# iaomw/Tracer

Hardware: AMD Instinct MI355X
Metric: Mrays/s at 1920x1080x64spp (higher is better)
Workload: dtype f32

## Files before the change

### include/tracer_test_hooks.h

```cpp
#ifndef TRACER_TEST_HOOKS_H
#define TRACER_TEST_HOOKS_H

#include "tracer_abi.h"

#ifdef __cplusplus
extern "C" {
#endif

trc_status trc_debug_profile(trc_ctx* ctx, uint64_t* out, uint32_t n_sites);
trc_status trc_sppm_hash_cells(trc_ctx* ctx, const float* cells , size_t n, float hash_scale, float* out );

trc_status trc_div_by_test(trc_ctx* ctx, const float* a, const float* b, size_t n, float* fast , float* plain );
trc_status trc_unary_test(trc_ctx* ctx, uint32_t op, uint32_t first_bits, uint64_t count, uint64_t* n_mismatch, uint32_t* first_mismatch);

trc_status trc_debug_denoise_state(trc_ctx* ctx, float* integrated, float* history, float* moments);

trc_status trc_texture_sample_test(trc_ctx* ctx, uint32_t index, const float* uv , size_t n, float* rgb );

trc_status trc_debug_env_tables(trc_ctx* ctx, float* weight, uint32_t* rows, uint32_t* marg, double* total, float* build_ms);
trc_status trc_env_light_test(trc_ctx* ctx, const uint32_t* draws , size_t n, float* dir_pdf ,
                              const float* dirs , size_t m, float* pdf );

trc_status trc_debug_mesh_light_tables(trc_ctx* ctx, uint32_t* alias , uint32_t* tri , float* pdfA ,
                                       double* total, uint32_t* n_lights);
trc_status trc_mesh_light_test(trc_ctx* ctx, const uint32_t* draws , const float* pos , size_t n, uint32_t* tri ,
                               float* out );

typedef struct trc_kernel_choice {
    uint32_t shape, variant, lds_resident, triangle_materials, strip, launches;
} trc_kernel_choice;
trc_status trc_debug_last_kernel(trc_ctx* ctx, trc_kernel_choice* out);


typedef struct trc_residency {
    uint32_t cu_count, block, waves, planned_per_cu, planned_with, per_cu;
    uint64_t lds_bytes;
    uint32_t lds_static_bytes, per_cu_block1280, dense_memo_rows, reserved;
} trc_residency;
trc_status trc_debug_last_residency(trc_ctx* ctx, trc_residency* out);

#ifdef __cplusplus
}
#endif
#endif
```

### tracer_amd/abi.py

```python
import ctypes as C

TRC_ABI_VERSION = 13
TRC_TILE = 16
TRC_MAX_BVH_DEPTH = 64
TREE_SAH, TREE_TRIANGLE_LEAVES = 1, 2
TRC_UNIQUE_ID_BYTES = 128
DT_U8, DT_U32, DT_F32 = 1, 3, 7
OP_SUM, OP_MAX, OP_MIN = 0, 2, 3

PRIM_SPHERE, PRIM_SQUARE, PRIM_CUBE, PRIM_TRIANGLE, PRIM_BVH, PRIM_UNKNOW = range(6)
(MAT_DIFFUSE, MAT_LAMBERT, MAT_ORENNAYAR, MAT_PLASTIC, MAT_METAL, MAT_GLASS,
 MAT_ISOTROPIC, MAT_DIELECTRIC, MAT_DEMOFOX, MAT_PBR, MAT_NIL) = range(11)
TEX_CONSTANT, TEX_CHECKER, TEX_NOISE, TEX_IMAGE = range(4)
INTEGRATOR_PATH, INTEGRATOR_MIS, INTEGRATOR_VOLUME = 0, 1, 2
MEDIUM_NIL, MEDIUM_HOMOGENEOUS, MEDIUM_GRIDDENSITY = 0, 1, 2
SCENE_CORNELL, SCENE_CORNELL_SPHERES, SCENE_CORNELL_MESH, SCENE_CORNELL_VOLUME = 0, 1, 2, 3
FLAG_COLLECT_STATS = 1
FLAG_FIXED_ORDER = 2
FLAG_SOBOL = 4
FLAG_SMALL_BLOCKS, FLAG_LARGE_BLOCKS = 8, 16
FLAG_ENV_LIGHT = 32
FLAG_MESH_LIGHTS = 64
TRACE_ANY_HIT, TRACE_PRODUCTION = 1, 2
SOBOL_DIMS, SOBOL_MATRIX_SIZE = 40, 52
# ... 174 lines not shown


class Hit(C.Structure):
    _fields_ = [("hit", C.c_int32), ("pType", C.c_int32), ("pIndex", C.c_uint32), ("t", C.c_float),
                ("p", C.c_float * 3), ("gn", C.c_float * 3), ("sn", C.c_float * 3), ("uv", C.c_float * 2),
                ("material", C.c_uint32), ("PDF", C.c_float),
                ("n_descend", C.c_uint32), ("n_return", C.c_uint32), ("n_leaf", C.c_uint32)]


class GBufferTexel(C.Structure):
    _fields_ = [("depth", C.c_float), ("normal", C.c_float * 3), ("albedo", C.c_float * 3), ("id", C.c_uint32)]


class DenoiseParams(C.Structure):
    _fields_ = [("flags", C.c_uint32), ("iterations", C.c_uint32), ("alpha_color", C.c_float), ("alpha_moments", C.c_float),
                ("sigma_z", C.c_float), ("normal_exponent", C.c_uint32), ("sigma_l", C.c_float), ("min_history", C.c_uint32)]


GBUFFER_MISS = 0xFFFFFFFF
DENOISE_DEMODULATE = 1
DENOISE_ALBEDO_EPS = 0.001
DENOISE_MAX_ITERATIONS = 5


class TreeCost(C.Structure):
    _fields_ = [("root_half_area", C.c_double), ("interior_half_area", C.c_double), ("leaf_half_area", C.c_double),
                ("n_interior", C.c_uint32), ("n_leaves", C.c_uint32)]


class KernelChoice(C.Structure):
    _fields_ = [("shape", C.c_uint32), ("variant", C.c_uint32), ("lds_resident", C.c_uint32), ("triangle_materials", C.c_uint32),
                ("strip", C.c_uint32), ("launches", C.c_uint32)]


class Residency(C.Structure):
    _fields_ = [("cu_count", C.c_uint32), ("block", C.c_uint32), ("waves", C.c_uint32), ("planned_per_cu", C.c_uint32),
                ("planned_with", C.c_uint32), ("per_cu", C.c_uint32), ("lds_bytes", C.c_uint64),
                ("lds_static_bytes", C.c_uint32), ("per_cu_block1280", C.c_uint32), ("dense_memo_rows", C.c_uint32), ("reserved", C.c_uint32)]


KERNEL_SHAPES = ("one", "strip", "pwg", "dense")
KERNEL_VARIANTS = ("plain", "stats", "sobol", "tex", "env", "env_tex", "mesh", "mesh_tex")


class LaunchShape(C.Structure):
    _fields_ = [("entries", C.c_uint32), ("wave_slots", C.c_uint32), ("longest_entry_ms", C.c_double),
                ("sum_entries_ms", C.c_double), ("work_over_slots_ms", C.c_double), ("clock_mhz", C.c_double)]


class Stats(C.Structure):
    _fields_ = [("paths", C.c_uint64), ("rays", C.c_uint64), ("shaded", C.c_uint64),
                ("n_descend", C.c_uint64), ("n_return", C.c_uint64),
                ("n_leaf_sphere", C.c_uint64), ("n_leaf_square", C.c_uint64),
                ("n_leaf_cube", C.c_uint64), ("n_leaf_triangle", C.c_uint64),
                ("n_hit_triangle", C.c_uint64), ("n_hit_cube", C.c_uint64),
                ("launches", C.c_uint64), ("kernel_ms", C.c_double), ("schedule_ms", C.c_double)]

    def as_dict(self):
        return {n: getattr(self, n) for n, _ in self._fields_}


_EXPECTED_SIZES = {float2: 8, float3: 16, float4x4: 64, AABB: 32, BVH: 64, Sphere: 272, Square: 272, Cube: 240,
                   TriangleVertex: 32, Pose: 144, SkinInfluence: 32, SkinBone: 128, MorphDelta: 24, TextureInfo: 32, Material: 64, Camera: 176, Ray: 32, Params: 32, GBufferTexel: 32, DenoiseParams: 32, TreeCost: 32,
                   PhotonRecord: 80, CameraRecord: 112, Complex: 96}
for _t, _n in _EXPECTED_SIZES.items():
    assert C.sizeof(_t) == _n, f"{_t.__name__}: ctypes size {C.sizeof(_t)} != ABI size {_n}"

DEVICE_SYMBOLS = [
    "trc_abi_version", "trc_build_flavor", "trc_has_test_hooks", "trc_status_string", "trc_last_error", "trc_create", "trc_destroy",
    "trc_upload_scene", "trc_upload_density", "trc_upload_scene_lbvh", "trc_upload_scene_sah", "trc_upload_scene_device", "trc_download_bvh", "trc_lbvh_info", "trc_set_camera", "trc_set_environment", "trc_set_environment_map", "trc_resize", "trc_seed",
    "trc_upload_rng", "trc_download_rng", "trc_upload_accum", "trc_download_accum", "trc_clear_accum", "trc_tonemap",
    "trc_render", "trc_synchronize", "trc_trace_rays", "trc_get_stats", "trc_reset_stats",
    "trc_sppm_init", "trc_sppm_frames", "trc_sppm_download",
    "trc_device_info", "trc_device_pci_bus_id", "trc_shard_seed", "trc_group_compose_samples", "trc_group_compose_samples_async", "trc_group_unique_id", "trc_group_init", "trc_group_reduce_accum", "trc_group_reduce_accum_async", "trc_group_allreduce_mean_accum", "trc_download_composed", "trc_group_finalize",
    "trc_group_set_collectives", "trc_debug_set", "trc_debug_block_costs", "trc_debug_launch_shape", "trc_debug_primary_replays",
    "trc_denoise_default_params", "trc_denoise", "trc_download_denoised", "trc_tonemap_denoised", "trc_download_gbuffer", "trc_denoise_reset",
    "trc_upload_textures", "trc_upload_triangle_materials", "trc_update_vertices", "trc_debug_refit_ms",
    "trc_pose_vertices", "trc_download_vertices", "trc_debug_pose_overflows", "trc_skin_bind", "trc_skin_vertices",
    "trc_morph_bind", "trc_morph_vertices", "trc_recompute_normals",
    "trc_rebuild_tree", "trc_tree_cost",
]
HOOK_SYMBOLS = ["trc_debug_profile", "trc_sppm_hash_cells", "trc_div_by_test", "trc_unary_test", "trc_debug_denoise_state", "trc_texture_sample_test",
                "trc_debug_env_tables", "trc_env_light_test", "trc_debug_mesh_light_tables", "trc_mesh_light_test", "trc_debug_last_kernel",
                "trc_debug_last_residency"]
HOST_SYMBOLS = [
    "trc_host_build_node", "trc_host_build_tree", "trc_host_tree_depth", "trc_host_make_camera",
    "trc_host_prepare_camera", "trc_host_fill_rng", "trc_host_scene_create", "trc_host_scene_create_leaves", "trc_host_scene_destroy",
    "trc_host_scene_view", "trc_host_scene_load_pbrt", "trc_host_mesh_load_obj", "trc_host_mesh_load_pbrt", "trc_host_mesh_load_ply", "trc_host_load_hdr", "trc_host_mesh_make_ball", "trc_host_mesh_replicate", "trc_host_mesh_from_arrays",
    "trc_host_mesh_view", "trc_host_mesh_destroy", "trc_host_make_density_info", "trc_host_make_cloud",
    "trc_host_load_density_pbrt", "trc_host_free", "trc_host_write_png", "trc_host_sobol_matrices32",
    "trc_host_sobol_interval_tables", "trc_host_load_png", "trc_host_scene_load_pbrt_flags", "trc_host_scene_triangle_materials",
]
```

### tracer_amd/csrc/dev_bsdf.hpp

```cpp
#pragma once

#include "dev_prof.hpp"
#include "dev_vec.hpp"

namespace trcdev {

TRC_DEV void coordinate_system(const F3 a, F3& b, F3& c) {
    if (fabsf(a.x) > fabsf(a.y)) b = f3(-a.z, 0, a.x);
    else b = f3(0, a.z, -a.y);
    b = normalize(b);
    c = cross(a, b);
}
TRC_DEV F2 concentric_sample_disk(const F2 u) {
    F2 uo; uo.x = 2.f * u.x - 1; uo.y = 2.f * u.y - 1;
    F2 r0; r0.x = 0; r0.y = 0;
    if (uo.x == 0 && uo.y == 0) return r0;
    const float PiOver2 = kPi / 2.0f, PiOver4 = kPi / 4.0f;
    const bool wide = fabsf(uo.x) > fabsf(uo.y);
    const float r = wide ? uo.x : uo.y;
    const float q = (wide ? uo.y : uo.x) / r;
    const float theta = wide ? PiOver4 * q : PiOver2 - PiOver4 * q;
    float s, c;
    dm_sincosf(theta, &s, &c);
    F2 out; out.x = r * c; out.y = r * s;
// ... 424 lines not shown
    const float etaA = 1.0f, etaB = 1.5f;
    bool live;
    bool pdf_live = false;
    bool f_live = false;
    F3 wi = wi_out, whA = wh, whB = wh;
    float eta = 0, fres_cos = 0, fres_eta = 1.5f;
    if (refl) {
        live = !(dot(wo, wh) <= 0);
        if (live) { wi = reflect(wo, wh); live = !(wo.z * wi.z <= 0); }
        if (live) {
            pdf_live = true;
            const float cosThetaO = abs_cos_theta(wo), cosThetaI = abs_cos_theta(wi);
            F3 sum = wi + wo;
            f_live = !(cosThetaI == 0 || cosThetaO == 0) && !(sum.x == 0 && sum.y == 0 && sum.z == 0);
            if (f_live) {
                whB = normalize(sum);
                const float d001 = whB.x * 0.0f + whB.y * 0.0f + whB.z * 1.0f;
                const F3 whf = (d001 < 0.f) ? -whB : whB;
                fres_cos = dot(wi, whf);
                fres_eta = 1.5f;
            }
        }
    } else {
        live = !(dot(wo, wh) < 0);
        if (live) live = refract(wo, wh, cos_theta(wo) > 0 ? (etaA / etaB) : (etaB / etaA), wi);
        if (live) {
            eta = cos_theta(wo) > 0 ? (etaB / etaA) : (etaA / etaB);
            const bool same_side = wo.z * wi.z > 0;
            whA = normalize(wo + wi * eta);
            const bool backfacing = dot(wo, whA) * dot(wi, whA) > 0;
            pdf_live = !same_side && !backfacing;
            whB = whA;
            if (whB.z < 0) whB = -whB;
            f_live = pdf_live && !(cos_theta(wi) == 0 || cos_theta(wo) == 0);
            fres_cos = dot(wo, whB);
            fres_eta = etaA;
        }
    }
    float D_A = 0, D_B = 0, lam_o = 0, lam_i = 0, fres = 0;
    if (pdf_live) {
        lam_o = d.lambda(wo);
        D_A = d.D(whA);
        D_B = D_A;
        if (refl && f_live) D_B = d.D(whB);
        if (f_live) {
            lam_i = d.lambda(wi);
            fres = fr_dielectric(fres_cos, fres_eta);
        }
    }
    F3 out = f3(0);
    if (live) {
        wi_out = wi;
        const float G1 = rcp1(1 + lam_o);
        const float G = rcp1(1 + lam_o + lam_i);
        if (refl) {
            const float dist_pdf = D_A * G1 * fabsf(dot(wo, wh)) / abs_cos_theta(wo);
            pdf_out = dist_pdf / (4 * dot(wo, wh));
            if (f_live) {
                const float cosThetaO = abs_cos_theta(wo), cosThetaI = abs_cos_theta(wi);
                out = f3(R) * D_B * G * f3(fres) / (4 * cosThetaI * cosThetaO);
            }
        } else {
            float p = 0;
            if (pdf_live) {
                const float sqrtDenom = dot(wo, whA) + eta * dot(wi, whA);
                const float dwh_dwi = fabsf((eta * eta * dot(wi, whA)) / (sqrtDenom * sqrtDenom));
                const float dist_pdf = D_A * G1 * fabsf(dot(wo, whA)) / abs_cos_theta(wo);
                p = dist_pdf * dwh_dwi;
            }
            pdf_out = p;
            if (f_live) {
                const float cosThetaO = cos_theta(wo), cosThetaI = cos_theta(wi);
                const float sqrtDenom = dot(wo, whB) + eta * dot(wi, whB);
                const float factor = 1;
                out = (f3(1.0f) - f3(fres)) * f3(0.98f) *
                      fabsf(D_B * G * eta * eta * fabsf(dot(wi, whB)) * fabsf(dot(wo, whB)) * factor * factor /
                            (cosThetaI * cosThetaO * sqrtDenom * sqrtDenom));
            }
        }
    }
    return out;
}

typedef MicroRefl<TrowbridgeReitzD<Alpha_01_02>, FrCond> MetalLobe;

constexpr int kMatDiffuse = 0, kMatLambert = 1, kMatPlastic = 3, kMatMetal = 4, kMatGlass = 5, kMatNil = 10;
constexpr int kTexConstant = 0, kTexChecker = 1, kTexImage = 3;

TRC_DEV F3 texture_value(int tex_type, F3 albedo, F2 uv) {
    if (tex_type == kTexChecker) {
        float s, c, s2, c2;
        dm_sincosf(8 * kPi * uv.x, &s, &c);
        dm_sincosf(kPi / 2 + 4 * kPi * uv.y, &s2, &c2);
        float sines = s * c2;
        return albedo * (0.5f * (sines < 0 ? 0.0f : 1.0f) + 0.5f);
    }
    return (tex_type >= 0 && tex_type <= 3) ? albedo : f3(1.0f);
}

template <bool STATS>
TRC_DEV F3 material_S_F(int type, F3 color, F3 wo, F3& wi, F2 uu, float& pdf, TravCounters& cnt) {
    const bool plastic = type == kMatPlastic, glass = type == kMatGlass;
    F3 out = f3(0);
    if (type == kMatMetal) {
        ProfScope<STATS> scope(cnt, kProfMetal);
        out = color * MetalLobe::S_F(1.0f, wo, wi, uu, pdf);
    } else if (type == kMatLambert || (plastic && uu.x < 0.5f)) {
        ProfScope<STATS> scope(cnt, kProfLambert);
        F2 u2 = uu;
        if (plastic) u2.x *= 2;
        const float v = Lambert::S_F(wo, wi, u2, pdf);
        out = plastic ? color * (f3(0.35f, 0.12f, 0.48f) * v) : color * f3(v);
    } else if (plastic || glass) {
        const float ratio = 0.25f;
        const bool refl = plastic || uu.x < ratio;
        F2 u2 = uu;
        if (plastic) { u2.x -= 0.5f; u2.x *= 2.0f; }
        else if (refl) u2.x = uu.x / ratio;
        else u2.x = (uu.x - ratio) / (1.0f - ratio);
        const Beckmann d = Beckmann::make_lobe(plastic);
        F3 lobe = f3(0);
        if (wo.z != 0) {
            F3 wh;
            { ProfScope<STATS> scope(cnt, kProfBeckSample); wh = d.sample_wh(wo, u2); }
            ProfScope<STATS> scope(cnt, kProfBeckEval);
            lobe = beckmann_finish(d, refl, plastic ? 1.0f : 0.98f, wo, wh, wi, pdf);
        }
        out = plastic ? color * (f3(0.2f) * lobe) : color * lobe;
    }
    return out;
}
TRC_DEV F3 material_S_F(int type, F3 color, F3 wo, F3& wi, F2 uu, float& pdf) {
    TravCounters none;
    return material_S_F<false>(type, color, wo, wi, uu, pdf, none);
}

TRC_DEV F3 material_F(int type, F3 color, F3 wo, F3 wi, F2 uu, float& pdf) {
    const bool plastic = type == kMatPlastic, glass = type == kMatGlass;
    if (type == kMatMetal) {
        pdf = MetalLobe::pdf(wo, wi);
        return color * MetalLobe::F(1.0f, wo, wi);
    }
    if (type == kMatLambert || (plastic && uu.x < 0.5f)) {
        pdf = Lambert::pdf(wo, wi);
        const float v = Lambert::F(wo, wi);
        return plastic ? color * (f3(0.35f, 0.12f, 0.48f) * v) : color * f3(v);
    }
    if (plastic || glass) {
        const float ratio = 0.25f;
        const Beckmann d = Beckmann::make_lobe(plastic);
        if (plastic || uu.x < ratio) {
            const float p = BeckRefl::pdf(d, wo, wi);
            pdf = plastic ? p : ratio * p;
            const F3 f = BeckRefl::F(d, plastic ? 1.0f : 0.98f, wo, wi);
            return plastic ? color * (f3(0.2f) * f) : color * f;
        }
        pdf = (1 - ratio) * BeckTransGlass::pdf(d, wo, wi);
        return color * BeckTransGlass::F(d, wo, wi);
    }
    pdf = 0;
    return f3(0);
}

}
```

### tracer_amd/csrc/trc_hooks.hip

```cpp
#include <hip/hip_runtime.h>

#include <string>

#include "trc_ctx.hpp"
#include "trc_render_config.hpp"

extern "C" int trc_has_test_hooks(void) {
#ifdef TRC_TEST_HOOKS
    return 1;
#else
    return 0;
#endif
}

#ifdef TRC_TEST_HOOKS
__global__ void __launch_bounds__(256) k_div_by_test(const float* a, const float* b, uint32_t n, float* fast, float* plain) {
    const uint32_t i = blockIdx.x * 256u + threadIdx.x;
    if (i >= n) return;
    const float av = a[i], bv = b[i];
    const GuardedDivBy d = guarded_div_by(bv);
    const F3 q = guarded_div(f3(av, -av, av * 0.75f), d);
    fast[3 * i] = q.x; fast[3 * i + 1] = q.y; fast[3 * i + 2] = q.z;
    plain[3 * i] = av / bv; plain[3 * i + 1] = -av / bv; plain[3 * i + 2] = (av * 0.75f) / bv;
}

__global__ void __launch_bounds__(256) k_unary_test(uint32_t op, uint32_t first, uint64_t count, unsigned long long* out) {
    unsigned long long bad = 0, first_bad = ~0ull;
    for (uint64_t i = (uint64_t)blockIdx.x * 256u + threadIdx.x; i < count; i += (uint64_t)gridDim.x * 256u) {
        const uint32_t bits = first + (uint32_t)i;
        const float x = __uint_as_float(bits);
        float a, b;
        if (op == 0u) { a = rcp_cr(x); b = 1.0f / x; }
        else if (op == 1u) { a = sqrt_cr(x); b = sqrtf(x); }
#if TRC_WAVE_GUARDS
        else if (op == 3u) { a = div_const(x, div_by_pi()); b = x / kPi; }
        else if (op == 4u) { a = div_const(x, div_by_sqr001()); b = x / (0.01f * 0.01f); }
        else if (op == 5u) { a = div_const(x, div_by_sqr002()); b = x / (0.02f * 0.02f); }
        else if (op == 6u) { a = div_const(x, div_by_sqr01()); b = x / (0.1f * 0.1f); }
#endif
        else { a = rsqrt_cr(x); b = 1.0f / sqrtf(x); }
        const bool same = __float_as_uint(a) == __float_as_uint(b) || (a != a && b != b);
        if (!same) { bad++; first_bad = min(first_bad, (unsigned long long)bits); }
    }
    if (bad) { atomicAdd(&out[0], bad); atomicMin(&out[1], first_bad); }
}

extern "C" {
trc_status trc_debug_profile(trc_ctx* ctx, uint64_t* out, uint32_t n_sites) {
    TRC_TRY(trc_flush(ctx));
    if (!ctx || !out) return TRC_ERR_INVALID_ARG;
    HIP_TRY(ctx, hipSetDevice(ctx->device));
    unsigned long long h[kStatCount + 3 * kProfCount];
    TRC_TRY(trc_read_stats_sum(ctx, h, kStatCount + 3 * kProfCount));
    for (uint32_t i = 0; i < n_sites && i < (uint32_t)kProfCount; ++i)
        for (int k = 0; k < 3; ++k) out[3 * i + k] = h[kStatCount + 3 * i + k];
    return TRC_OK;
}

__global__ void __launch_bounds__(256) k_texture_sample_test(const float* texels, const uint4* desc, uint32_t n_tex, uint32_t index,
                                                             const float* uv, uint32_t n, float* rgb) {
    const uint32_t i = blockIdx.x * 256u + threadIdx.x;
    if (i >= n) return;
    TexTable tt; tt.texels = texels; tt.desc = desc; tt.n = n_tex;
    F2 p; p.x = uv[2 * i]; p.y = uv[2 * i + 1];
    const F3 c = image_sample(tt, index, p);
    rgb[3 * i] = c.x; rgb[3 * i + 1] = c.y; rgb[3 * i + 2] = c.z;
}
trc_status trc_texture_sample_test(trc_ctx* ctx, uint32_t index, const float* uv, size_t n, float* rgb) {
    TRC_TRY(trc_flush(ctx));
    if (!ctx || (n && (!uv || !rgb))) return TRC_ERR_INVALID_ARG;
    if (index >= ctx->n_tex) return trc_fail(ctx, TRC_ERR_INVALID_ARG, "trc_texture_sample_test: no such image");
    if (n == 0) return TRC_OK;
    if (n > 0x7FFFFFFFu / 3u) return trc_fail(ctx, TRC_ERR_INVALID_ARG, "trc_texture_sample_test: too many pairs in one call");
    HIP_TRY(ctx, hipSetDevice(ctx->device));
    DevBuf d;
    TRC_TRY(d.alloc(ctx, n * 5 * sizeof(float), "texture sample test"));
    float *d_uv = d.as<float>(), *d_rgb = d_uv + 2 * n;
    TRC_TRY(trc_copy_to_device(ctx, d_uv, uv, n * 8, ctx->stream));
    hipLaunchKernelGGL(k_texture_sample_test, dim3((unsigned)((n + 255) / 256)), dim3(256), 0, ctx->stream,
                       ctx->d_tex_texels, ctx->d_tex_desc, ctx->n_tex, index, d_uv, (uint32_t)n, d_rgb);
    const hipError_t e = hipGetLastError();
    if (e != hipSuccess) return trc_fail(ctx, TRC_ERR_HIP, std::string("trc_texture_sample_test: ") + hipGetErrorString(e));
    return trc_copy_to_host(ctx, rgb, d_rgb, n * 12, ctx->stream);
}

trc_status trc_debug_last_kernel(trc_ctx* ctx, trc_kernel_choice* out) {
    TRC_TRY(trc_flush(ctx));
    if (!ctx || !out) return TRC_ERR_INVALID_ARG;
    const trc_ctx::LastKernel& k = ctx->last_kernel;
    out->shape = k.shape; out->variant = k.variant; out->lds_resident = k.lds_resident; out->triangle_materials = k.tri_materials;
    out->strip = k.strip; out->launches = k.count;
    return TRC_OK;
}
trc_status trc_debug_last_residency(trc_ctx* ctx, trc_residency* out) {
    TRC_TRY(trc_flush(ctx));
    if (!ctx || !out) return TRC_ERR_INVALID_ARG;
    const trc_ctx::LastFit& f = ctx->last_fit;
    *out = trc_residency{};
    if (!f.fn) return TRC_OK;
    HIP_TRY(ctx, hipSetDevice(ctx->device));
    int now = 0;
    HIP_TRY(ctx, hipOccupancyMaxActiveBlocksPerMultiprocessor(&now, f.fn, (int)f.block, f.lds));
    hipFuncAttributes attr{};
    HIP_TRY(ctx, hipFuncGetAttributes(&attr, f.fn));
    out->cu_count = (uint32_t)ctx->cu_count; out->block = f.block; out->waves = f.waves; out->planned_per_cu = f.planned_per_cu;
    out->planned_with = f.per_cu; out->per_cu = now > 0 ? (uint32_t)now : 0u; out->lds_bytes = (uint64_t)f.lds;
    out->lds_static_bytes = (uint32_t)attr.sharedSizeBytes;
    out->per_cu_block1280 = trc_lds_workgroups((uint32_t)(f.lds + attr.sharedSizeBytes), 1280u, 160u * 1024u);
    out->dense_memo_rows = ctx->last_kernel.shape == 3u ? (uint32_t)TRC_REPLAY_DENSE : 0u;
    return TRC_OK;
}

trc_status trc_div_by_test(trc_ctx* ctx, const float* a, const float* b, size_t n, float* fast, float* plain) {
    if (!ctx || (n && (!a || !b || !fast || !plain))) return TRC_ERR_INVALID_ARG;
    if (n == 0) return TRC_OK;
    if (n > 0x7FFFFFFFu / 3u) return trc_fail(ctx, TRC_ERR_INVALID_ARG, "trc_div_by_test: too many pairs in one call");
    HIP_TRY(ctx, hipSetDevice(ctx->device));
    DevBuf d;
    TRC_TRY(d.alloc(ctx, n * 8 * sizeof(float), "div_by test"));
    float *d_a = d.as<float>(), *d_b = d_a + n, *d_fast = d_a + 2 * n, *d_plain = d_a + 5 * n;
    TRC_TRY(trc_copy_to_device(ctx, d_a, a, n * 4, ctx->stream));
    TRC_TRY(trc_copy_to_device(ctx, d_b, b, n * 4, ctx->stream));
    hipLaunchKernelGGL(k_div_by_test, dim3((unsigned)((n + 255) / 256)), dim3(256), 0, ctx->stream, d_a, d_b, (uint32_t)n, d_fast, d_plain);
    const hipError_t e = hipGetLastError();
    if (e != hipSuccess) return trc_fail(ctx, TRC_ERR_HIP, std::string("trc_div_by_test: ") + hipGetErrorString(e));
    TRC_TRY(trc_copy_to_host(ctx, fast, d_fast, n * 12, ctx->stream));
    return trc_copy_to_host(ctx, plain, d_plain, n * 12, ctx->stream);
}

trc_status trc_unary_test(trc_ctx* ctx, uint32_t op, uint32_t first_bits, uint64_t count, uint64_t* n_mismatch, uint32_t* first_mismatch) {
    if (!ctx || !n_mismatch || op > 6u || count > (1ull << 32)) return TRC_ERR_INVALID_ARG;
    HIP_TRY(ctx, hipSetDevice(ctx->device));
    DevBuf buf;
    TRC_TRY(buf.alloc(ctx, 16, "unary test"));
    unsigned long long* const d = buf.as<unsigned long long>();
    unsigned long long h[2] = {0ull, ~0ull};
    TRC_TRY(trc_copy_to_device(ctx, d, h, 16, ctx->stream));
    if (count) hipLaunchKernelGGL(k_unary_test, dim3(ctx->cu_count * 16), dim3(256), 0, ctx->stream, op, first_bits, count, d);
    TRC_TRY(trc_read_to_host(ctx, ctx->stream, "trc_unary_test", {{h, d, 16}}));
    *n_mismatch = h[0];
    if (first_mismatch) *first_mismatch = (uint32_t)h[1];
    return TRC_OK;
}

}
#endif
```

### tracer_amd/csrc/trc_render_lds.hip

```cpp
#ifndef TRC_TRIANGLE_MATERIALS
#define TRC_TRIANGLE_MATERIALS 0
#endif
#ifndef TRC_FAST_UNARY
#define TRC_FAST_UNARY 1
#endif
#include "trc_render_kernels.hpp"

TRC_RENDER_NS_BEGIN
__global__ void __launch_bounds__(kBlock, TRC_PATH_WAVES_DENSE) k_render_dense(const KRender kp) {
    render_workgroup<true, false, TRC_INTEGRATOR_PATH, false, TRC_PARK_DENSE, false, Light::None, TRC_REPLAY_DENSE, TRC_REPLAY_DENSE_GLOBAL != 0>(kp);
}

const RenderKernels render_lds_path = render_kernels<true, TRC_INTEGRATOR_PATH>();
const RenderKernel render_dense = render_kernel(&k_render_dense, TRC_PATH_WAVES_DENSE);
TRC_RENDER_NS_END
```

### tracer_amd/csrc/trc_render_lds_mis.hip

```cpp
#ifndef TRC_TRIANGLE_MATERIALS
#define TRC_TRIANGLE_MATERIALS 0
#endif
#ifndef TRC_FAST_UNARY
#define TRC_FAST_UNARY 1
#endif
#include "trc_render_kernels.hpp"

TRC_RENDER_NS_BEGIN
const RenderKernels render_lds_mis = render_kernels<true, TRC_INTEGRATOR_MIS>();
const RenderKernels render_lds_volume = render_kernels<true, TRC_INTEGRATOR_VOLUME>();
TRC_RENDER_NS_END
```

### tracer_amd/device.py

```python
import ctypes as C
import os

import numpy as np

from . import abi

_LIB = None
_LIB_FAST = None
_LIB_HOOKS = None


class TracerError(RuntimeError):
    def __init__(self, what, status, detail=""):
        super().__init__(f"{what}: trc_status {status}" + (f" ({detail})" if detail else ""))
        self.status = status


def lib_path():
    return os.environ.get("TRC_AMD_LIB") or os.path.join(os.path.dirname(os.path.abspath(__file__)), "lib", "libtracer_amd.so")


def fast_lib_path():
    return os.path.join(os.path.dirname(os.path.abspath(__file__)), "lib", "libtracer_amd_fast.so")

# ... 28 lines not shown
    L.trc_abi_version.restype = u32
    L.trc_build_flavor.restype = C.c_char_p
    L.trc_status_string.argtypes = [i32]
    L.trc_status_string.restype = C.c_char_p
    L.trc_last_error.argtypes = [vp]
    L.trc_last_error.restype = C.c_char_p
    L.trc_create.argtypes = [C.c_int, C.POINTER(vp)]
    L.trc_destroy.argtypes = [vp]
    L.trc_destroy.restype = None
    L.trc_upload_scene.argtypes = [vp, C.POINTER(abi.Scene)]
    L.trc_set_environment_map.argtypes = [vp, u32, u32, vp]
    L.trc_tonemap.argtypes = [vp, vp, C.POINTER(C.c_float)]
    L.trc_upload_density.argtypes = [vp, C.POINTER(abi.GridDensityInfo), vp]
    L.trc_upload_scene_lbvh.argtypes = [vp, C.POINTER(abi.Scene)]
    L.trc_upload_scene_sah.argtypes = [vp, C.POINTER(abi.Scene)]
    L.trc_upload_scene_device.argtypes = [vp, C.POINTER(abi.Scene), u32]
    L.trc_download_bvh.argtypes = [vp, C.POINTER(abi.BVH), u32, C.POINTER(u32)]
    L.trc_lbvh_info.argtypes = [vp, C.POINTER(u32), C.POINTER(u32), C.POINTER(C.c_float)]
    L.trc_set_camera.argtypes = [vp, C.POINTER(abi.Camera)]
    L.trc_set_environment.argtypes = [vp, C.POINTER(C.c_float)]
    L.trc_resize.argtypes = [vp, u32, u32]
    L.trc_seed.argtypes = [vp, u64]
    for name in ("trc_upload_rng", "trc_download_rng", "trc_upload_accum", "trc_download_accum"):
        getattr(L, name).argtypes = [vp, vp]
    L.trc_clear_accum.argtypes = [vp]
    L.trc_render.argtypes = [vp, C.POINTER(abi.Params)]
    L.trc_synchronize.argtypes = [vp]
    L.trc_trace_rays.argtypes = [vp, vp, C.c_size_t, vp, C.c_int]
    L.trc_get_stats.argtypes = [vp, C.POINTER(abi.Stats)]
    L.trc_reset_stats.argtypes = [vp]
    L.trc_sppm_init.argtypes = [vp, u64]
    L.trc_sppm_frames.argtypes = [vp, u32]
    L.trc_sppm_download.argtypes = [vp, vp, vp, vp, vp, C.POINTER(abi.Complex)]
    L.trc_device_info.argtypes = [vp, C.c_char_p, C.c_size_t, C.POINTER(C.c_int), C.POINTER(C.c_size_t)]
    L.trc_group_unique_id.argtypes = [C.POINTER(C.c_uint8)]
    L.trc_group_init.argtypes = [vp, C.POINTER(C.c_uint8), C.c_int, C.c_int]
    L.trc_group_reduce_accum.argtypes = [vp, C.c_int]
    L.trc_group_reduce_accum_async.argtypes = [vp, C.c_int]
    L.trc_group_allreduce_mean_accum.argtypes = [vp]
    L.trc_group_compose_samples.argtypes = [vp, C.c_int, u32]
    L.trc_group_compose_samples_async.argtypes = [vp, C.c_int, u32]
    L.trc_shard_seed.argtypes = [u64, u32]
    L.trc_device_pci_bus_id.argtypes = [vp, C.c_char_p, C.c_size_t]
    L.trc_download_composed.argtypes = [vp, vp]
    L.trc_group_finalize.argtypes = [vp]
    L.trc_group_set_collectives.argtypes = [vp, vp, C.c_int, C.c_int]
    L.trc_debug_set.argtypes = [vp, C.c_char_p, C.c_int]
    L.trc_debug_block_costs.argtypes = [vp, vp, vp, u32, C.POINTER(u32), C.POINTER(u32)]
    L.trc_debug_launch_shape.argtypes = [vp, C.POINTER(abi.LaunchShape)]
    L.trc_debug_primary_replays.argtypes = [vp, C.POINTER(u64)]
    L.trc_denoise_default_params.argtypes = [C.POINTER(abi.DenoiseParams)]
    L.trc_denoise.argtypes = [vp, C.POINTER(abi.DenoiseParams)]
    L.trc_download_denoised.argtypes = [vp, vp]
    L.trc_tonemap_denoised.argtypes = [vp, vp, C.POINTER(C.c_float)]
    L.trc_download_gbuffer.argtypes = [vp, vp]
    L.trc_denoise_reset.argtypes = [vp]
    L.trc_upload_textures.argtypes = [vp, C.POINTER(abi.Image), u32]
    L.trc_upload_triangle_materials.argtypes = [vp, vp, u32]
    L.trc_update_vertices.argtypes = [vp, vp, u32, u32]
    L.trc_debug_refit_ms.argtypes = [vp, C.POINTER(C.c_float)]
    L.trc_pose_vertices.argtypes = [vp, C.POINTER(abi.Pose), u32]
    L.trc_download_vertices.argtypes = [vp, vp, u32, u32]
    L.trc_debug_pose_overflows.argtypes = [vp, C.POINTER(u32)]
    L.trc_skin_bind.argtypes = [vp, vp, u32, u32]
    L.trc_skin_vertices.argtypes = [vp, C.POINTER(abi.SkinBone), u32]
    L.trc_morph_bind.argtypes = [vp, vp, u32, u32, u32]
    L.trc_morph_vertices.argtypes = [vp, vp, u32, C.POINTER(abi.SkinBone), u32]
    L.trc_recompute_normals.argtypes = [vp, u32, u32]
    L.trc_rebuild_tree.argtypes = [vp, u32]
    L.trc_tree_cost.argtypes = [vp, C.POINTER(abi.TreeCost)]
    if hooks:
        L.trc_debug_profile.argtypes = [vp, C.POINTER(C.c_uint64), u32]
        L.trc_sppm_hash_cells.argtypes = [vp, vp, C.c_size_t, C.c_float, vp]
        L.trc_div_by_test.argtypes = [vp, vp, vp, C.c_size_t, vp, vp]
        L.trc_unary_test.argtypes = [vp, u32, u32, C.c_uint64, C.POINTER(C.c_uint64), C.POINTER(u32)]
        L.trc_debug_denoise_state.argtypes = [vp, vp, vp, vp]
        L.trc_texture_sample_test.argtypes = [vp, u32, vp, C.c_size_t, vp]
        L.trc_debug_env_tables.argtypes = [vp, vp, vp, vp, C.POINTER(C.c_double), C.POINTER(C.c_float)]
        L.trc_env_light_test.argtypes = [vp, vp, C.c_size_t, vp, vp, C.c_size_t, vp]
        L.trc_debug_mesh_light_tables.argtypes = [vp, vp, vp, vp, C.POINTER(C.c_double), C.POINTER(u32)]
        L.trc_mesh_light_test.argtypes = [vp, vp, vp, C.c_size_t, vp, vp]
        L.trc_debug_last_kernel.argtypes = [vp, C.POINTER(abi.KernelChoice)]
        L.trc_debug_last_residency.argtypes = [vp, C.POINTER(abi.Residency)]
        for name in abi.HOOK_SYMBOLS:
            getattr(L, name).restype = i32
    L.trc_has_test_hooks.restype = C.c_int
    for name in abi.DEVICE_SYMBOLS:
        f = getattr(L, name)
        if name not in ("trc_abi_version", "trc_build_flavor", "trc_has_test_hooks", "trc_status_string", "trc_last_error", "trc_destroy", "trc_shard_seed",
                        "trc_denoise_default_params"):
            f.restype = i32
    L.trc_shard_seed.restype = u64
    L.trc_denoise_default_params.restype = None
    if L.trc_abi_version() != abi.TRC_ABI_VERSION:
        raise RuntimeError("libtracer_amd.so ABI version mismatch")
    return L


def make_poses(poses):
    arr = (abi.Pose * len(poses))()
    for k, (first, count, model, normal) in enumerate(poses):
        arr[k].first, arr[k].count = int(first), int(count)
        for name, m in (("model_matrix", model), ("normal_matrix", normal)):
            m = np.asarray(m, dtype=np.float32).reshape(4, 4)
            cols = getattr(arr[k], name).columns
            for c in range(4):
                cols[c].x, cols[c].y, cols[c].z, cols[c].w = (float(m[r, c]) for r in range(4))
    return arr


def make_bones(palette):
    m = np.asarray(palette, dtype=np.float32).reshape(-1, 2, 4, 4)
    cols = np.ascontiguousarray(m.transpose(0, 1, 3, 2))
    return (abi.SkinBone * len(cols)).from_buffer_copy(cols.tobytes())


def group_unique_id():
    buf = (C.c_uint8 * abi.TRC_UNIQUE_ID_BYTES)()
    st = lib().trc_group_unique_id(buf)
    if st != abi.OK:
        raise TracerError("trc_group_unique_id", st)
    return bytes(buf)


class Tracer:

    def __init__(self, device=0, fast_math=False, hooks=False):
        self._L = lib(fast_math, hooks)
        self._env_shape = (0, 0)
        self._h = C.c_void_p()
        st = self._L.trc_create(device, C.byref(self._h))
        if st != abi.OK:
            self._h = None
            raise TracerError(f"trc_create(device={device})", st, self._L.trc_status_string(st).decode())
        self.width = self.height = 0
        self._n_vertex = 0

    def _check(self, st, what):
        if st != abi.OK:
            raise TracerError(what, st, self._L.trc_last_error(self._h).decode())

    def close(self):
        if getattr(self, "_h", None):
            self._L.trc_destroy(self._h)
            self._h = None

    __del__ = close

    def __enter__(self):
        return self

    def __exit__(self, *exc):
        self.close()

    def upload_scene(self, scene_view):
        self._check(self._L.trc_upload_scene(self._h, C.byref(scene_view)), "trc_upload_scene")
        self._n_vertex = scene_view.n_vertex

    def set_environment_map(self, rgb):
        if rgb is None:
            self._check(self._L.trc_set_environment_map(self._h, 0, 0, None), "trc_set_environment_map")
            self._env_shape = (0, 0)
            return
        assert rgb.dtype == np.float32 and rgb.ndim == 3 and rgb.shape[2] == 3 and rgb.flags.c_contiguous
        self._check(self._L.trc_set_environment_map(self._h, rgb.shape[1], rgb.shape[0], rgb.ctypes.data),
                    "trc_set_environment_map")
# ... 284 lines not shown

    def reset_stats(self):
        self._check(self._L.trc_reset_stats(self._h), "trc_reset_stats")

    def device_info(self):
        name = C.create_string_buffer(256)
        cu, mem = C.c_int(), C.c_size_t()
        self._check(self._L.trc_device_info(self._h, name, 256, C.byref(cu), C.byref(mem)), "trc_device_info")
        return {"name": name.value.decode(), "cu_count": cu.value, "hbm_bytes": mem.value}

    def sppm_init(self, photon_seed):
        self._check(self._L.trc_sppm_init(self._h, photon_seed), "trc_sppm_init")

    def sppm_frames(self, n_frames=1):
        self._check(self._L.trc_sppm_frames(self._h, n_frames), "trc_sppm_frames")

    def sppm_hash_cells(self, cells, hash_scale):
        cells = np.ascontiguousarray(cells, dtype=np.float32).reshape(-1, 3)
        out = np.empty(len(cells), dtype=np.float32)
        self._check(self._L.trc_sppm_hash_cells(self._h, cells.ctypes.data, len(cells), float(hash_scale), out.ctypes.data),
                    "trc_sppm_hash_cells")
        return out

    def sppm_download(self):
        from .dtypes import CAMREC_DTYPE, PHOTON_DTYPE
        n = abi.PHOTON_HASHN
        cam = np.zeros(self.width * self.height, dtype=CAMREC_DTYPE)
        pho = np.zeros(n * n, dtype=PHOTON_DTYPE)
        mark = np.zeros((n, n, 4), dtype=np.float32)
        count = np.zeros((n, n), dtype=np.float32)
        cx = abi.Complex()
        self._check(self._L.trc_sppm_download(self._h, cam.ctypes.data, pho.ctypes.data, mark.ctypes.data,
                                              count.ctypes.data, C.byref(cx)), "trc_sppm_download")
        return cam, pho, mark, count, cx

    def group_init(self, unique_id, nranks, rank):
        buf = (C.c_uint8 * abi.TRC_UNIQUE_ID_BYTES).from_buffer_copy(unique_id)
        self._check(self._L.trc_group_init(self._h, buf, nranks, rank), "trc_group_init")

    def group_reduce_accum(self, root=0):
        self._check(self._L.trc_group_reduce_accum(self._h, root), "trc_group_reduce_accum")

    def group_allreduce_mean_accum(self):
        self._check(self._L.trc_group_allreduce_mean_accum(self._h), "trc_group_allreduce_mean_accum")

    def group_compose_samples(self, root=0, sample_groups=None):
        self._check(self._L.trc_group_compose_samples(self._h, root, sample_groups or 0), "trc_group_compose_samples")

    def group_compose_samples_async(self, root=0, sample_groups=None):
        self._check(self._L.trc_group_compose_samples_async(self._h, root, sample_groups or 0), "trc_group_compose_samples_async")

    def pci_bus_id(self):
        buf = C.create_string_buffer(64)
        self._check(self._L.trc_device_pci_bus_id(self._h, buf, 64), "trc_device_pci_bus_id")
        return buf.value.decode()

    def group_reduce_accum_async(self, root=0):
        self._check(self._L.trc_group_reduce_accum_async(self._h, root), "trc_group_reduce_accum_async")

    def download_composed(self):
        out = np.empty((self.height, self.width, 4), dtype=np.float32)
        self._check(self._L.trc_download_composed(self._h, out.ctypes.data), "trc_download_composed")
        return out

    def set_collectives(self, table, nranks, rank):
        self._coll = table
        self._check(self._L.trc_group_set_collectives(self._h, C.byref(table.table) if table is not None else None, nranks, rank),
                    "trc_group_set_collectives")

    def debug_set(self, knob, value):
        self._check(self._L.trc_debug_set(self._h, knob.encode(), int(value)), "trc_debug_set")

    def last_kernel(self):
        k = abi.KernelChoice()
        self._check(self._L.trc_debug_last_kernel(self._h, C.byref(k)), "trc_debug_last_kernel")
        return dict(shape=abi.KERNEL_SHAPES[k.shape], variant=abi.KERNEL_VARIANTS[k.variant], lds_resident=bool(k.lds_resident),
                    triangle_materials=bool(k.triangle_materials), strip=int(k.strip), launches=int(k.launches))

    def last_residency(self):
        r = abi.Residency()
        self._check(self._L.trc_debug_last_residency(self._h, C.byref(r)), "trc_debug_last_residency")
        return {name: int(getattr(r, name)) for name, _ in abi.Residency._fields_}

    def div_by_test(self, a, b):
        a = np.ascontiguousarray(a, dtype=np.float32); b = np.ascontiguousarray(b, dtype=np.float32)
        assert a.shape == b.shape and a.ndim == 1
        fast, plain = np.empty((len(a), 3), np.float32), np.empty((len(a), 3), np.float32)
        self._check(self._L.trc_div_by_test(self._h, a.ctypes.data, b.ctypes.data, len(a), fast.ctypes.data, plain.ctypes.data), "trc_div_by_test")
        return fast, plain

    def block_costs(self):
        n, bs = C.c_uint32(0), C.c_uint32(0)
        self._check(self._L.trc_debug_block_costs(self._h, None, None, 0, C.byref(n), C.byref(bs)), "trc_debug_block_costs")
        tiles, costs = np.zeros(n.value, np.uint32), np.zeros(n.value, np.uint32)
        self._check(self._L.trc_debug_block_costs(self._h, tiles.ctypes.data, costs.ctypes.data, n.value, C.byref(n), C.byref(bs)),
                    "trc_debug_block_costs")
        return tiles, costs, bs.value

    def unary_test(self, op, first_bits=0, count=1 << 32):
        n, first = C.c_uint64(0), C.c_uint32(0)
        self._check(self._L.trc_unary_test(self._h, op, first_bits, count, C.byref(n), C.byref(first)), "trc_unary_test")
        return n.value, first.value

    def launch_shape(self):
        s = abi.LaunchShape()
        self._check(self._L.trc_debug_launch_shape(self._h, C.byref(s)), "trc_debug_launch_shape")
        return {k: getattr(s, k) for k, _ in abi.LaunchShape._fields_}

    def primary_replays(self):
        n = C.c_uint64(0)
        self._check(self._L.trc_debug_primary_replays(self._h, C.byref(n)), "trc_debug_primary_replays")
        return n.value

    def group_finalize(self):
        self._check(self._L.trc_group_finalize(self._h), "trc_group_finalize")
```

Measured before the change: 15040.

## Unify microfacet material lobes into one runtime-parameterized sampling path

Adds a single Microfacet struct whose roughness and distribution (Trowbridge-Reitz or Beckmann) are chosen at runtime. material_S_F uses it for metal, plastic and glass in the non-stats LDS render kernels, replacing separate templated lobe instantiations. The aim is less code and branch divergence, and possibly lower register pressure, when different materials share a wavefront. The cost is runtime selects and extra arithmetic inside every lobe, and results could drift numerically from the templated path; a test hook is added to compare the two.

```diff
diff --git a/include/tracer_test_hooks.h b/include/tracer_test_hooks.h
--- a/include/tracer_test_hooks.h
+++ b/include/tracer_test_hooks.h
@@ -12,6 +12,9 @@
 
 trc_status trc_div_by_test(trc_ctx* ctx, const float* a, const float* b, size_t n, float* fast , float* plain );
 trc_status trc_unary_test(trc_ctx* ctx, uint32_t op, uint32_t first_bits, uint64_t count, uint64_t* n_mismatch, uint32_t* first_mismatch);
+
+trc_status trc_material_s_f_test(trc_ctx* ctx, uint32_t stream, const uint32_t* type , const float* color ,
+                                 const float* wo , const float* uu , size_t n, float pdf_init, float* out );
 
 trc_status trc_debug_denoise_state(trc_ctx* ctx, float* integrated, float* history, float* moments);
 
diff --git a/tracer_amd/abi.py b/tracer_amd/abi.py
--- a/tracer_amd/abi.py
+++ b/tracer_amd/abi.py
@@ -280,7 +280,7 @@
 ]
 HOOK_SYMBOLS = ["trc_debug_profile", "trc_sppm_hash_cells", "trc_div_by_test", "trc_unary_test", "trc_debug_denoise_state", "trc_texture_sample_test",
                 "trc_debug_env_tables", "trc_env_light_test", "trc_debug_mesh_light_tables", "trc_mesh_light_test", "trc_debug_last_kernel",
-                "trc_debug_last_residency"]
+                "trc_debug_last_residency", "trc_material_s_f_test"]
 HOST_SYMBOLS = [
     "trc_host_build_node", "trc_host_build_tree", "trc_host_tree_depth", "trc_host_make_camera",
     "trc_host_prepare_camera", "trc_host_fill_rng", "trc_host_scene_create", "trc_host_scene_create_leaves", "trc_host_scene_destroy",
diff --git a/tracer_amd/csrc/dev_bsdf.hpp b/tracer_amd/csrc/dev_bsdf.hpp
--- a/tracer_amd/csrc/dev_bsdf.hpp
+++ b/tracer_amd/csrc/dev_bsdf.hpp
@@ -530,6 +530,225 @@
     return out;
 }
 
+#ifndef TRC_MICROFACET_STREAM
+#define TRC_MICROFACET_STREAM 0
+#endif
+
+struct Microfacet {
+    bool tr;
+    float alpha_x, alpha_y;
+    DivConst by_ax2, by_ay2;
+    TRC_DEV static Microfacet make_lobe(bool metal, bool plastic) {
+        Microfacet d; d.tr = metal;
+        d.alpha_x = fmaxf(0.001f, 0.01f); d.alpha_y = fmaxf(0.001f, metal ? 0.02f : plastic ? 0.1f : 0.01f);
+        d.by_ax2 = div_by_sqr001();
+        const DivConst rough = div_by_sqr01(), mid = div_by_sqr002(), smooth = div_by_sqr001();
+        d.by_ay2.c = metal ? mid.c : plastic ? rough.c : smooth.c; d.by_ay2.y = metal ? mid.y : plastic ? rough.y : smooth.y;
+        return d;
+    }
+    TRC_DEV float ax() const { return alpha_x; }
+    TRC_DEV float ay() const { return alpha_y; }
+
+    TRC_DEV float lambda(F3 w) const {
+        const float st = sin_theta(w);
+        const Phi ph = phi_of(w, st);
+        const float zz = w.z * w.z;
+        const float temp = 1 - zz;
+        const float num = tr ? temp : st, den = tr ? zz : w.z;
+        const float t = (temp <= 0.0f || den == 0.0f) ? 0.0f : num / den;
+        const float x = tr ? 1 + (sqr(ph.c * ax()) + sqr(ph.s * ay())) * t
+                           : (ph.c * ph.c) * ax() * ax() + (ph.s * ph.s) * ay() * ay();
+        const float r = sqrt_cr(x);
+        if (is_inf(t)) return 0.;
+        if (tr) return 0.5f * (r - 1);
+        float a = rcp1(r * fabsf(t));
+        if (a >= 1.6f) return 0;
+        return (1 - 1.259f * a + 0.396f * a * a) / (3.535f * a + 2.181f * a * a);
+    }
+    TRC_DEV float D(F3 wh) const {
+        float tan2Theta = tan2_theta(wh);
+        if (is_inf(tan2Theta)) return 0.;
+        const float cos4Theta = cos2_theta(wh) * cos2_theta(wh);
+        if (tr && cos4Theta < 1e-16f) return 0;
+        const Phi ph = phi_of(wh);
+        float qc, qs;
+        div_const2(ph.c * ph.c, by_ax2, ph.s * ph.s, by_ay2, qc, qs);
+        if (tr) {
+            float e = (qc + qs) * tan2Theta;
+            return rcp1(kPi * ax() * ay() * sqr(1 + e) * cos4Theta);
+        }
+        return dm_expf(-tan2Theta * (qc + qs)) /
+               (kPi * ax() * ay() * cos4Theta);
+    }
+
+    TRC_DEV void sample11(float cosTheta, float sinTheta, float U1, float U2, float& slope_x, float& slope_y) const {
+        if (cosTheta > .9999f) {
+            float r2;
+            if (tr) r2 = U1 / (1 - U1);
+            else r2 = -dm_logf(1.0f - U1);
+            float r = sqrt_cr(r2);
+            const float phi = tr ? 6.28318530718f * U2 : 2 * kPi * U2;
+            float s, c;
+            dm_sincosf(phi, &s, &c);
+            slope_x = r * c;
+            slope_y = r * s;
+            return;
+        }
+        const float tanTheta = sinTheta / cosTheta;
+        const float cotTheta = rcp1(tanTheta);
+        if (tr) {
+            const float a = cotTheta;
+            float G1 = 2 * rcp1(1 + sqrt_cr(1.f + rcp1(a * a)));
+            float A = 2 * U1 / G1 - 1;
+            float tmp = rcp1(A * A - 1.f);
+            if (tmp > 1e10f) tmp = 1e10f;
+            float B = tanTheta;
+            float D = sqrt_cr(fmaxf(B * B * tmp * tmp - (A * A - B * B) * tmp, 0.0f));
+            float slope_x_1 = B * tmp - D;
+            float slope_x_2 = B * tmp + D;
+            slope_x = (A < 0 || slope_x_2 > a) ? slope_x_1 : slope_x_2;
+            float S;
+            if (U2 > 0.5f) { S = 1.f; U2 = 2.f * (U2 - .5f); }
+            else { S = -1.f; U2 = 2.f * (.5f - U2); }
+            float z = (U2 * (U2 * (U2 * 0.27385f - 0.73369f) + 0.46341f)) /
+                      (U2 * (U2 * (U2 * 0.093073f + 0.309420f) - 1.000000f) + 0.597999f);
+            slope_y = S * z * sqrt_cr(1.f + slope_x * slope_x);
+            return;
+        }
+        const float tanThetaI = tanTheta, cotThetaI = cotTheta, cosThetaI = cosTheta;
+        float a = -1, c = erf_approx(cotThetaI);
+        float sample_x = fmaxf(U1, 1e-6f);
+        float thetaI = dm_acosf(cosThetaI);
+        float fit = 1 + thetaI * (-0.876f + thetaI * (0.4265f - 0.0594f * thetaI));
+        const float base = 1 - sample_x;
+        const float pw = dm_expf_fin(fit * dm_logf_pos(base == 0.0f ? 1.0f : base));
+        float b = c - (1 + c) * (base == 0.0f ? 0.0f : pw);
+        const float SQRT_PI_INV = 1.f / sqrtf(kPi);
+        float normalization = rcp1(1 + c + SQRT_PI_INV * tanThetaI * dm_expf(-cotThetaI * cotThetaI));
+        int it = 0;
+        while (++it < 10) {
+            if (!(b >= a && b <= c)) b = 0.5f * (a + c);
+            float invErf = erf_inv(b);
+            float value = normalization * (1 + b + SQRT_PI_INV * tanThetaI * dm_expf_fin(-invErf * invErf)) - sample_x;
+            float derivative = normalization * (1 - invErf * tanThetaI);
+            if (fabsf(value) < 1e-5f) break;
+            if (value > 0) c = b; else a = b;
+            b -= value / derivative;
+        }
+        slope_x = erf_inv(b);
+        slope_y = erf_inv(2.0f * fmaxf(U2, 1e-6f) - 1.0f);
+    }
+    TRC_DEV F3 sample_wh(F3 wo, F2 u) const {
+        const bool flip = wo.z < 0;
+        const F3 wi = flip ? -wo : wo;
+        F3 wiStretched = normalize(f3(ax() * wi.x, ay() * wi.y, wi.z));
+        float slope_x, slope_y;
+        const float st = sin_theta(wiStretched);
+        sample11(cos_theta(wiStretched), st, u.x, u.y, slope_x, slope_y);
+        const Phi ph = phi_of(wiStretched, st);
+        float tmp = ph.c * slope_x - ph.s * slope_y;
+        slope_y = ph.s * slope_x + ph.c * slope_y;
+        slope_x = tmp;
+        slope_x = ax() * slope_x;
+        slope_y = ay() * slope_y;
+        F3 wh = normalize(f3(-slope_x, -slope_y, 1.f));
+        return flip ? -wh : wh;
+    }
+};
+
+TRC_DEV F3 microfacet_finish(const Microfacet& d, bool refl, float R, F3 wo, F3 wh, F3& wi_out, float& pdf_out) {
+    const float etaA = 1.0f, etaB = 1.5f;
+    bool live;
+    bool pdf_live = false;
+    bool f_live = false;
+    F3 wi = wi_out, whA = wh, whB = wh;
+    float eta = 0, fres_cos = 0, fres_eta = 1.5f;
+    if (refl) {
+        live = !(dot(wo, wh) <= 0);
+        if (live) {
+            wi = reflect(wo, wh);
+            if (d.tr) wi_out = wi;
+            live = !(wo.z * wi.z <= 0);
+        }
+        if (live) {
+            pdf_live = true;
+            const float cosThetaO = abs_cos_theta(wo), cosThetaI = abs_cos_theta(wi);
+            F3 sum = wi + wo;
+            f_live = !(cosThetaI == 0 || cosThetaO == 0) && !(sum.x == 0 && sum.y == 0 && sum.z == 0);
+            if (f_live) {
+                whB = normalize(sum);
+                const float d001 = whB.x * 0.0f + whB.y * 0.0f + whB.z * 1.0f;
+                const F3 whf = (d001 < 0.f) ? -whB : whB;
+                fres_cos = dot(wi, whf);
+                fres_eta = 1.5f;
+            }
+        }
+    } else {
+        live = !(dot(wo, wh) < 0);
+        if (live) live = refract(wo, wh, cos_theta(wo) > 0 ? (etaA / etaB) : (etaB / etaA), wi);
+        if (live) {
+            eta = cos_theta(wo) > 0 ? (etaB / etaA) : (etaA / etaB);
+            const bool same_side = wo.z * wi.z > 0;
+            whA = normalize(wo + wi * eta);
+            const bool backfacing = dot(wo, whA) * dot(wi, whA) > 0;
+            pdf_live = !same_side && !backfacing;
+            whB = whA;
+            if (whB.z < 0) whB = -whB;
+            f_live = pdf_live && !(cos_theta(wi) == 0 || cos_theta(wo) == 0);
+            fres_cos = dot(wo, whB);
+            fres_eta = etaA;
+        }
+    }
+    float D_A = 0, D_B = 0, lam_o = 0, lam_i = 0;
+    F3 fres = f3(0);
+    if (pdf_live) {
+        lam_o = d.lambda(wo);
+        D_A = d.D(whA);
+        D_B = D_A;
+        if (refl && f_live) D_B = d.D(whB);
+        if (f_live) {
+            lam_i = d.lambda(wi);
+            if (d.tr) fres = FrCond::eval(fres_cos);
+            else fres = f3(fr_dielectric(fres_cos, fres_eta));
+        }
+    }
+    F3 out = f3(0);
+    if (live) {
+        wi_out = wi;
+        const float G1 = rcp1(1 + lam_o);
+        const float G = rcp1(1 + lam_o + lam_i);
+        if (refl) {
+            const float dwh = dot(wo, wh);
+            const float num = d.tr ? dwh : D_A * G1 * fabsf(dwh), den = d.tr ? cos_theta(wo) : abs_cos_theta(wo);
+            const float q = num / den;
+            const float dist_pdf = d.tr ? D_A * G1 * fabsf(q) : q;
+            pdf_out = dist_pdf / (4 * dot(wo, wh));
+            if (f_live) {
+                const float cosThetaO = abs_cos_theta(wo), cosThetaI = abs_cos_theta(wi);
+                out = f3(R) * D_B * G * fres / (4 * cosThetaI * cosThetaO);
+            }
+        } else {
+            float p = 0;
+            if (pdf_live) {
+                const float sqrtDenom = dot(wo, whA) + eta * dot(wi, whA);
+                const float dwh_dwi = fabsf((eta * eta * dot(wi, whA)) / (sqrtDenom * sqrtDenom));
+                const float dist_pdf = D_A * G1 * fabsf(dot(wo, whA)) / abs_cos_theta(wo);
+                p = dist_pdf * dwh_dwi;
+            }
+            pdf_out = p;
+            if (f_live) {
+                const float cosThetaO = cos_theta(wo), cosThetaI = cos_theta(wi);
+                const float sqrtDenom = dot(wo, whB) + eta * dot(wi, whB);
+                const float factor = 1;
+                out = (f3(1.0f) - fres) * f3(0.98f) *
+                      fabsf(D_B * G * eta * eta * fabsf(dot(wi, whB)) * fabsf(dot(wo, whB)) * factor * factor /
+                            (cosThetaI * cosThetaO * sqrtDenom * sqrtDenom));
+            }
+        }
+    }
+    return out;
+}
+
 typedef MicroRefl<TrowbridgeReitzD<Alpha_01_02>, FrCond> MetalLobe;
 
 constexpr int kMatDiffuse = 0, kMatLambert = 1, kMatPlastic = 3, kMatMetal = 4, kMatGlass = 5, kMatNil = 10;
@@ -546,10 +765,35 @@
     return (tex_type >= 0 && tex_type <= 3) ? albedo : f3(1.0f);
 }
 
-template <bool STATS>
+template <bool STATS, bool STREAM = (TRC_MICROFACET_STREAM != 0)>
 TRC_DEV F3 material_S_F(int type, F3 color, F3 wo, F3& wi, F2 uu, float& pdf, TravCounters& cnt) {
     const bool plastic = type == kMatPlastic, glass = type == kMatGlass;
     F3 out = f3(0);
+    if constexpr (STREAM && !STATS) {
+        const bool metal = type == kMatMetal;
+        if (type == kMatLambert || (plastic && uu.x < 0.5f)) {
+            F2 u2 = uu;
+            if (plastic) u2.x *= 2;
+            const float v = Lambert::S_F(wo, wi, u2, pdf);
+            out = plastic ? color * (f3(0.35f, 0.12f, 0.48f) * v) : color * f3(v);
+        } else if (metal || plastic || glass) {
+            const float ratio = 0.25f;
+            const bool refl = metal || plastic || uu.x < ratio;
+            F2 u2 = uu;
+            if (metal) { }
+            else if (plastic) { u2.x -= 0.5f; u2.x *= 2.0f; }
+            else if (refl) u2.x = uu.x / ratio;
+            else u2.x = (uu.x - ratio) / (1.0f - ratio);
+            const Microfacet d = Microfacet::make_lobe(metal, plastic);
+            F3 lobe = f3(0);
+            if (wo.z != 0) {
+                const F3 wh = d.sample_wh(wo, u2);
+                lobe = microfacet_finish(d, refl, (metal || plastic) ? 1.0f : 0.98f, wo, wh, wi, pdf);
+            }
+            out = plastic ? color * (f3(0.2f) * lobe) : color * lobe;
+        }
+        return out;
+    }
     if (type == kMatMetal) {
         ProfScope<STATS> scope(cnt, kProfMetal);
         out = color * MetalLobe::S_F(1.0f, wo, wi, uu, pdf);
diff --git a/tracer_amd/csrc/trc_hooks.hip b/tracer_amd/csrc/trc_hooks.hip
--- a/tracer_amd/csrc/trc_hooks.hip
+++ b/tracer_amd/csrc/trc_hooks.hip
@@ -43,6 +43,21 @@
         if (!same) { bad++; first_bad = min(first_bad, (unsigned long long)bits); }
     }
     if (bad) { atomicAdd(&out[0], bad); atomicMin(&out[1], first_bad); }
+}
+
+template <bool STREAM>
+__global__ void __launch_bounds__(256) k_material_s_f_test(const uint32_t* type, const float* color, const float* wo, const float* uu,
+                                                           uint32_t n, float pdf_init, float* out) {
+    const uint32_t i = blockIdx.x * 256u + threadIdx.x;
+    if (i >= n) return;
+    F2 u; u.x = uu[2 * i]; u.y = uu[2 * i + 1];
+    F3 wi = f3(0);
+    float pdf = pdf_init;
+    TravCounters none;
+    const F3 f = material_S_F<false, STREAM>((int)type[i], f3(color[3 * i], color[3 * i + 1], color[3 * i + 2]),
+                                             f3(wo[3 * i], wo[3 * i + 1], wo[3 * i + 2]), wi, u, pdf, none);
+    float* o = out + 7 * (size_t)i;
+    o[0] = wi.x; o[1] = wi.y; o[2] = wi.z; o[3] = f.x; o[4] = f.y; o[5] = f.z; o[6] = pdf;
 }
 
 extern "C" {
@@ -128,6 +143,28 @@
     return trc_copy_to_host(ctx, plain, d_plain, n * 12, ctx->stream);
 }
 
+trc_status trc_material_s_f_test(trc_ctx* ctx, uint32_t stream, const uint32_t* type, const float* color, const float* wo, const float* uu,
+                                 size_t n, float pdf_init, float* out) {
+    if (!ctx || stream > 1u || (n && (!type || !color || !wo || !uu || !out))) return TRC_ERR_INVALID_ARG;
+    if (n == 0) return TRC_OK;
+    if (n > 0x7FFFFFFFu / 7u) return trc_fail(ctx, TRC_ERR_INVALID_ARG, "trc_material_s_f_test: too many inputs in one call");
+    HIP_TRY(ctx, hipSetDevice(ctx->device));
+    DevBuf d;
+    TRC_TRY(d.alloc(ctx, n * 16 * sizeof(float), "material S_F test"));
+    float *d_color = d.as<float>(), *d_wo = d_color + 3 * n, *d_uu = d_color + 6 * n, *d_out = d_color + 8 * n;
+    uint32_t* d_type = reinterpret_cast<uint32_t*>(d_color + 15 * n);
+    TRC_TRY(trc_copy_to_device(ctx, d_color, color, n * 12, ctx->stream));
+    TRC_TRY(trc_copy_to_device(ctx, d_wo, wo, n * 12, ctx->stream));
+    TRC_TRY(trc_copy_to_device(ctx, d_uu, uu, n * 8, ctx->stream));
+    TRC_TRY(trc_copy_to_device(ctx, d_type, type, n * 4, ctx->stream));
+    const dim3 grid((unsigned)((n + 255) / 256));
+    if (stream) hipLaunchKernelGGL(k_material_s_f_test<true>, grid, dim3(256), 0, ctx->stream, d_type, d_color, d_wo, d_uu, (uint32_t)n, pdf_init, d_out);
+    else hipLaunchKernelGGL(k_material_s_f_test<false>, grid, dim3(256), 0, ctx->stream, d_type, d_color, d_wo, d_uu, (uint32_t)n, pdf_init, d_out);
+    const hipError_t e = hipGetLastError();
+    if (e != hipSuccess) return trc_fail(ctx, TRC_ERR_HIP, std::string("trc_material_s_f_test: ") + hipGetErrorString(e));
+    return trc_copy_to_host(ctx, out, d_out, n * 28, ctx->stream);
+}
+
 trc_status trc_unary_test(trc_ctx* ctx, uint32_t op, uint32_t first_bits, uint64_t count, uint64_t* n_mismatch, uint32_t* first_mismatch) {
     if (!ctx || !n_mismatch || op > 6u || count > (1ull << 32)) return TRC_ERR_INVALID_ARG;
     HIP_TRY(ctx, hipSetDevice(ctx->device));
diff --git a/tracer_amd/csrc/trc_render_lds.hip b/tracer_amd/csrc/trc_render_lds.hip
--- a/tracer_amd/csrc/trc_render_lds.hip
+++ b/tracer_amd/csrc/trc_render_lds.hip
@@ -3,6 +3,9 @@
 #endif
 #ifndef TRC_FAST_UNARY
 #define TRC_FAST_UNARY 1
+#endif
+#ifndef TRC_MICROFACET_STREAM
+#define TRC_MICROFACET_STREAM 1
 #endif
 #include "trc_render_kernels.hpp"
 
diff --git a/tracer_amd/csrc/trc_render_lds_mis.hip b/tracer_amd/csrc/trc_render_lds_mis.hip
--- a/tracer_amd/csrc/trc_render_lds_mis.hip
+++ b/tracer_amd/csrc/trc_render_lds_mis.hip
@@ -3,6 +3,9 @@
 #endif
 #ifndef TRC_FAST_UNARY
 #define TRC_FAST_UNARY 1
+#endif
+#ifndef TRC_MICROFACET_STREAM
+#define TRC_MICROFACET_STREAM 1
 #endif
 #include "trc_render_kernels.hpp"
 
diff --git a/tracer_amd/device.py b/tracer_amd/device.py
--- a/tracer_amd/device.py
+++ b/tracer_amd/device.py
@@ -134,6 +134,7 @@
         L.trc_mesh_light_test.argtypes = [vp, vp, vp, C.c_size_t, vp, vp]
         L.trc_debug_last_kernel.argtypes = [vp, C.POINTER(abi.KernelChoice)]
         L.trc_debug_last_residency.argtypes = [vp, C.POINTER(abi.Residency)]
+        L.trc_material_s_f_test.argtypes = [vp, u32, vp, vp, vp, vp, C.c_size_t, C.c_float, vp]
         for name in abi.HOOK_SYMBOLS:
             getattr(L, name).restype = i32
     L.trc_has_test_hooks.restype = C.c_int
@@ -584,6 +585,16 @@
         self._check(self._L.trc_debug_last_residency(self._h, C.byref(r)), "trc_debug_last_residency")
         return {name: int(getattr(r, name)) for name, _ in abi.Residency._fields_}
 
+    def material_s_f_test(self, types, color, wo, uu, stream, pdf_init=0.0):
+        types = np.ascontiguousarray(types, dtype=np.uint32)
+        color, wo, uu = (np.ascontiguousarray(a, dtype=np.float32) for a in (color, wo, uu))
+        n = len(types)
+        assert types.ndim == 1 and color.shape == (n, 3) and wo.shape == (n, 3) and uu.shape == (n, 2)
+        out = np.empty((n, 7), np.float32)
+        self._check(self._L.trc_material_s_f_test(self._h, 1 if stream else 0, types.ctypes.data, color.ctypes.data, wo.ctypes.data,
+                                                  uu.ctypes.data, n, float(pdf_init), out.ctypes.data), "trc_material_s_f_test")
+        return out
+
     def div_by_test(self, a, b):
         a = np.ascontiguousarray(a, dtype=np.float32); b = np.ascontiguousarray(b, dtype=np.float32)
         assert a.shape == b.shape and a.ndim == 1
```

Result: faster. 15690, median of 6 (+4.3%).
